# slcs-jsc/mptrac

Hardware: AMD Instinct MI355X
Metric: particle-steps/s (higher is better)
Workload: dtype f64

## Files before the change

### mptrac_amd/csrc/mphip_api.hip

```cpp
#include <hip/hip_runtime.h>
#include <dlfcn.h>
#include <unistd.h>

#include <algorithm>
#include <atomic>
#include <cmath>
#include <cstdio>
#include <cstring>
#include <string>
#include <mutex>
#include <thread>
#include <vector>

#include "mphip_buffers.hpp"
#include "mphip_kernels.hpp"
#include "mphip_metprep.hpp"
#include "mphip_regrid.hpp"
#include "mphip_detrend.hpp"
#include "mphip_ingest.hpp"
#include "mphip_pack.hpp"
#include "mphip_intpol.hpp"

using namespace mphip;

namespace {

constexpr unsigned kAdv = MPHIP_MOD_TIMESTEPS | MPHIP_MOD_POSITION | MPHIP_MOD_ADVECT | MPHIP_MOD_POSITION2;
constexpr unsigned kAdvTurb = kAdv | MPHIP_MOD_DIFF_TURB;
constexpr unsigned kAdvDiff = kAdvTurb | MPHIP_MOD_DIFF_MESO;
constexpr unsigned kAdvTurbConvSedi = kAdvTurb | MPHIP_MOD_CONVECTION | MPHIP_MOD_SEDI;
constexpr unsigned kAdvDiffConvSedi = kAdvDiff | MPHIP_MOD_CONVECTION | MPHIP_MOD_SEDI;
constexpr unsigned kDiffConvSediOnly = MPHIP_MOD_TIMESTEPS | MPHIP_MOD_DIFF_TURB | MPHIP_MOD_DIFF_MESO | MPHIP_MOD_CONVECTION
  | MPHIP_MOD_SEDI | MPHIP_MOD_POSITION2;
constexpr unsigned kTailOnly = MPHIP_MOD_TIMESTEPS;
constexpr unsigned kBound = MPHIP_MOD_BOUND_COND | MPHIP_MOD_BOUND_COND2;
constexpr unsigned kParticleBits = 0x3fffu | MPHIP_MOD_ISOSURF | kBound | MPHIP_MOD_ISOSURF_INIT;

const char *const kField3Name[MPHIP_N3D] = { "u", "v", "w", "t", "lwc", "rwc", "iwc", "swc", "pl", "ul", "vl", "zetal",
                                             "zeta_dotl", "h2o", "z", "pv", "o3", "cc", "wl" };
const char *const kField2Name[MPHIP_N2D] = { "ps", "pbl", "cape", "cin", "pel", "pct", "pcb", "cl", "ess", "nss", "shf", "ts",
                                             "zs", "us", "vs", "lsm", "sst", "pt", "tt", "zt", "h2ot", "plcl", "plfc", "o3c" };
// ... 69 lines not shown
    bool ml_monotonic = false;
    DevBuf<float> meso;
    bool meso_valid = false;
  };
  PackedGrids pk, pk_next;
  bool pk_next_valid = false;
  bool packed_dirty = true;

  long long np = 0, ip0 = 0, np_total = 0;
  int nq = 0;
  DevBuf<double> d_arr[4 + MPHIP_NQ_MAX];
  DevBuf<double> d_alt[4 + MPHIP_NQ_MAX];
  DevBuf<float> d_uvwp[3], d_uvwp_alt[3];
  DevBuf<double> d_dt, d_dt_alt;
  uint64_t rng_ctr = 0;
  DevBuf<double> d_iso, d_iso_alt;
  DevBuf<int> d_kz, d_kz_alt;
  DevBuf<double> d_iso_ts, d_iso_ps;
  int iso_n = 0;
  std::vector<std::pair<uintptr_t, uintptr_t>> pinned;
  std::mutex pinned_lock;

  DevBuf<int> d_ext, d_ext_alt;
  bool ext_identity = true;
  int steps_since_resort = 1 << 30;
  const int *fold_perm = nullptr;
  DevBuf<f32x4u> d_prec;

  DevBuf<uint32_t> d_keys[2];
  DevBuf<int> d_vals[2];
  DevBuf<uint32_t> d_counts;
  int sorted_buf = -1;
  const int *fused_perm = nullptr;
  bool fused_quantities = false;
  bool stored_is_sorted = false;
  long long sorted_n = 0;
  DevBuf<uint32_t> rep_sk, rep_mk[2], rep_fk, rep_tiles, rep_nm;
  DevBuf<int> rep_si, rep_mi[2], rep_fv;
  hipStream_t ahead_stream = nullptr;
  hipEvent_t ahead_mark = nullptr, ahead_done = nullptr;
  DevBuf<uint32_t> ahead_keys[2];
  DevBuf<int> ahead_vals[2];
  DevBuf<uint32_t> ahead_counts;
  DevBuf<double> ahead_dt;
  bool ahead_valid = false;
  double ahead_t = 0;
  int ahead_cur = 0;
  bool ahead_repaired = false;
  long long sorts_repaired = 0, sorts_scratch = 0;
  long long sorts_undone = 0;
  DevBuf<unsigned char> d_depo_busy;
  bool depo_busy_valid = false;
  const unsigned char *depo_busy_last = nullptr;
  unsigned depo_busy_last_mask = 0;

  DevBuf<int> d_cell;
  DevBuf<double> d_sums;
  DevBuf<int> d_cnt;
  DevBuf<unsigned long long> d_lists;
  DevBuf<double> d_rec;
  PinnedBuf<double> h_sums;
  DevBuf<double> d_grid_kernel;
  int grid_nk = 0;

  DevBuf<double> d_chemgrid;
  bool chemgrid_ok = false;
// ... 5 lines not shown
  RadioQnt radio = { { -1, -1, -1, -1, -1, -1 } };
  bool radio_on = false;
  bool rdepo_on = false;
  mphip_box_t rdepo_grid = {};
  DevBuf<double> d_rdepo_inv;
  size_t rdepo_ntot = 0;
  bool rdepo_have_t = false;
  double rdepo_t = 0;

  DevBuf<double> d_ana_kernel;
  DevBuf<uint32_t> d_marks;
  DevBuf<int> d_slot_of;
  DevBuf<uint32_t> d_ana_flags;

  mphip_allreduce_fn allreduce = nullptr;
  void *allreduce_user = nullptr;
  void *comm = nullptr;
  int comm_ranks = 1, comm_rank = 0;
  DevBuf<double> d_occ, d_band;
  PinnedBuf<double> h_occ;
  DevBuf<int> d_band_cnt;
  int mix_band_lo = -1, mix_band_hi = -1;

  PrepState prep;

  DevBuf<double> d_ip_in, d_ip_out;

  int locality_interval = 60;
  bool locality_zorder = false;
  int locality_tile = 0;
  int step_blocks = 8192;
  int step_blocks_multi = 32768;
  bool xcd_map = true;
  bool big_grid = false;
  bool force_generic = false;
  int multi_step = 64;
  bool fold_resort = true;
  int lds_tile = 0;
  bool turb_strat = true;
  bool compact_depo = true;
  bool pin_host_atm = false;
  bool perm_records = true;
  bool fuse_sort = true;
  bool fuse_quantities = true;
  int sort_bits = 0;
  bool sort_repair = true;
  bool sort_ahead = true;
  bool ahead_box = true;
  bool ahead_priority = false;
  bool emit_keys = true;
  int deterministic_sums = 1;
  int sum_path = 0;
  bool grid_records = true;
  int chain_blocks = 0;
  bool mix_exchange_levels = false;
  int derive_profile_phase = 0;
  int intpol_chunk = 1 << 22;

  bool prof = false;
  std::vector<hipEvent_t> ev;
  size_t ev_used = 0;
};

namespace {

int fail(mphip_ctx *ctx, const std::string &msg) {
// ... 654 lines not shown
      sel = kAdvDiffConvSedi | kGated | scheme | multi;
  } else if (!(rare_bits & ~kBound) && big_ok && (req & ~kOptionalModules) == kAdv) {
    sel = kAdvDiffConvSedi | kGated | kBigGrid | scheme | multi;
  }
#ifdef MPHIP_QUICK
  if (sel != kAdvDiffConvSedi && sel != (kAdvDiffConvSedi | kMultiStep) && sel != (kAdvDiffConvSedi | kMLWinds | kMultiStep)
      && sel != (kAdvDiffConvSedi | kGated | kPblClosure | kMultiStep))
    sel = kNoStepKernel;
#endif
  if (sel != kNoStepKernel)
    return sel;
  if (ml_fast)
    return nsteps > 1 ? kMaskGenericMLMulti : kMaskGenericML;
  if (nsteps > 1)
    return kNoStepKernel;
  return ml || (mask & kRareModules) || fg ? kMaskGeneric : kMaskGenericPL;
}

static bool reads_meso_table(unsigned sel, unsigned mask) {
  return sel != kNoStepKernel && sel < kMaskGenericMLMulti && (sel & MPHIP_MOD_DIFF_MESO)
    && !(sel & kBigGrid) && (mask & MPHIP_MOD_DIFF_MESO);
}

int ensure_meso_table(mphip_ctx *ctx) {
  mphip_ctx::PackedGrids &K = ctx->pk;
  if (K.meso_valid)
    return 0;
  HIPCHK(K.meso.reserve(meso_table_floats(ctx)));
  if (meso_table_launch(ctx, K, ctx->stream))
    return fail(ctx, "building the table of the mesoscale wind deviations failed");
  return 0;
}

int launch_step(mphip_ctx *ctx, unsigned mask, double t, const RngCtr &rng = {}, int nsteps = 1, double t_stride = 0,
                uint64_t ctr_stride = 0, const EmitKeys *emit = nullptr, bool *emitted = nullptr) {
  if (ctx->np == 0)
    return 0;
  if (ensure_packed(ctx) || check_fields(ctx, mask))
    return 1;
  if (ml_winds(ctx->ctl) && !ctx->d_kz.p) {
    const size_t n = (size_t) std::max<long long>(ctx->np, 1);
    HIPCHK(ctx->d_kz.resize(n));
    HIPCHK(ctx->d_kz_alt.resize(n));
    std::vector<int> mid(n, std::max(ctx->nml / 2, 0));
    HIPCHK(hipMemcpyAsync(ctx->d_kz.p, mid.data(), n * sizeof(int), hipMemcpyHostToDevice, ctx->stream));
    HIPCHK(hipStreamSynchronize(ctx->stream));
  }
  StepParams S;
  memset(&S.emit, 0, sizeof(S.emit));
  S.depo_busy = nullptr;
  if (emitted)
    *emitted = false;
  S.ctl = ctx->ctl;
  S.met = dev_met(ctx);
  S.atm = dev_atm(ctx);
  S.clim = ctx->d_clim.p;
  S.tracers = ctx->d_tracers.p;
  S.t = t;
  S.mask = mask;
  const BlockGeom geom = block_geom(ctx->np, nsteps > 1 ? ctx->step_blocks_multi : ctx->step_blocks);
  const int nb = geom.nblocks_logical;
  const long long per_block = geom.per_block;
  S.nblocks_logical = nb;
  S.per_block = per_block;
  S.xcd_map = ctx->xcd_map;
  S.ctr_turb = rng.turb;
  S.ctr_meso = rng.meso;
  S.ctr_conv = rng.conv;
  S.ctr_pbl = rng.pbl;
  S.radio = ctx->radio;
  S.nsteps = nsteps;
  S.t_stride = t_stride;
  S.ctr_stride = ctr_stride;
  size_t lds = axes_lds_bytes(ctx) + sizeof(DevClim) + (size_t) kLibmLogExpDoubles * sizeof(double);
  hipEvent_t e1 = nullptr;
  if (prof_pair(ctx, ctx->stream, &e1))
    return 1;
  unsigned sel = step_kernel_mask(ctx, mask, nsteps);
  if (reads_meso_table(sel, mask)) {
    if (ensure_meso_table(ctx))
      return 1;
    S.met.meso = ctx->pk.meso.p;
  }
  constexpr unsigned kDepo = MPHIP_MOD_WET_DEPO | MPHIP_MOD_DRY_DEPO;
  const size_t depo_lds = ((axes_lds_bytes(ctx) + 15) & ~(size_t) 15) + (size_t) per_block * sizeof(int);
  if (sel == kTailOnly && (mask & kDepo) && !(mask & ~kDepo) && ctx->compact_depo && !ctx->fused_perm
      && depo_lds <= 64 * 1024) {
    S.depo_busy = ctx->depo_busy_valid ? ctx->d_depo_busy.p : nullptr;
    ctx->depo_busy_valid = false;
    ctx->depo_busy_last = S.depo_busy;
    ctx->depo_busy_last_mask = mask;
    hipLaunchKernelGGL(depo_kernel, dim3(nb), dim3(256), depo_lds, ctx->stream, S);
    HIPCHK(hipGetLastError());
    ctx->fused_perm = nullptr;
    if (ctx->prof)
      HIPCHK(hipEventRecord(e1, ctx->stream));
    return 0;
  }
  ctx->depo_busy_valid = false;
  ctx->depo_busy_last = nullptr;
  if (emit && emit->keys && sel == kAdvDiffConvSedi && nsteps == 1) {
    sel |= kEmitKeys;
    S.emit = *emit;
    if (emitted)
      *emitted = true;
    ctx->depo_busy_valid = emit->depo_busy != nullptr;
  }
  if (ctx->lds_tile > 0 && nsteps > 1 && (sel == (kAdv | kMultiStep) || sel == (kAdv | kTwoStage | kMultiStep))
      && !(mask & (kTailModules | kBound)) && !ctx->fused_perm) {
    const size_t tile_lds = ((axes_lds_bytes(ctx) + 15) & ~(size_t) 15) + (size_t) ctx->lds_tile * 24;
    if (tile_lds <= 64 * 1024) {
      if (sel & kTwoStage)
        hipLaunchKernelGGL(traj_tile_kernel<2>, dim3(nb), dim3(256), tile_lds, ctx->stream, S, ctx->lds_tile);
      else
        hipLaunchKernelGGL(traj_tile_kernel<4>, dim3(nb), dim3(256), tile_lds, ctx->stream, S, ctx->lds_tile);
      HIPCHK(hipGetLastError());
      if (ctx->prof)
        HIPCHK(hipEventRecord(e1, ctx->stream));
      return 0;
    }
  }
  if (sel < kMaskGenericMLMulti && (sel & kPblClosure))
    lds += (size_t) (kLibmDoubles - kLibmLogExpDoubles) * sizeof(double);
  if (step_kernel_parks(sel))
    lds += kParkBytes;
  switch (sel) {
#define STEP_CASE(M)                                                                                  \
  case M:                                                                                             \
    hipLaunchKernelGGL(step_kernel<M>, dim3(nb), dim3(256), lds, ctx->stream, S);                     \
    break;
#ifdef MPHIP_QUICK
#define STEP_CASE_REST(M)
#else
#define STEP_CASE_REST(M) STEP_CASE(M)
#endif
    STEP_CASE_REST(kAdv)
    STEP_CASE_REST(kAdvTurb)
    STEP_CASE_REST(kAdvDiff)
    STEP_CASE_REST(kAdvTurbConvSedi)
    STEP_CASE(kAdvDiffConvSedi)
    STEP_CASE_REST(kAdv | kTwoStage)
    STEP_CASE_REST(kAdvTurb | kTwoStage)
    STEP_CASE_REST(kAdvDiff | kTwoStage)
    STEP_CASE_REST(kAdvTurbConvSedi | kTwoStage)
    STEP_CASE_REST(kAdvDiffConvSedi | kTwoStage)
    STEP_CASE_REST(kAdvDiffConvSedi | kGated)
    STEP_CASE_REST(kAdvDiffConvSedi | kGated | kTwoStage)
    STEP_CASE_REST(kTailOnly)
    STEP_CASE_REST(kDiffConvSediOnly)
    STEP_CASE_REST(kAdv | kMultiStep)
    STEP_CASE_REST(kAdvTurb | kMultiStep)
    STEP_CASE_REST(kAdvDiff | kMultiStep)
    STEP_CASE(kAdvDiffConvSedi | kMultiStep)
    STEP_CASE_REST(kAdvDiffConvSedi | kMLWinds)
    STEP_CASE(kAdvDiffConvSedi | kMLWinds | kMultiStep)
    STEP_CASE_REST(kAdvDiffConvSedi | kGated | kMLWinds)
    STEP_CASE_REST(kAdvDiffConvSedi | kGated | kMLWinds | kMultiStep)
    STEP_CASE_REST(kAdv | kTwoStage | kMultiStep)
    STEP_CASE_REST(kAdvTurb | kTwoStage | kMultiStep)
    STEP_CASE_REST(kAdvDiff | kTwoStage | kMultiStep)
    STEP_CASE_REST(kAdvDiffConvSedi | kTwoStage | kMultiStep)
    STEP_CASE_REST(kAdvDiffConvSedi | kGated | kMultiStep)
    STEP_CASE_REST(kAdvDiffConvSedi | kGated | kTwoStage | kMultiStep)
    STEP_CASE(kAdvDiffConvSedi | kEmitKeys)
    STEP_CASE_REST(kAdvDiffConvSedi | kGated | kPblClosure)
    STEP_CASE_REST(kAdvDiffConvSedi | kGated | kPblClosure | kTwoStage)
    STEP_CASE(kAdvDiffConvSedi | kGated | kPblClosure | kMultiStep)
    STEP_CASE_REST(kAdvDiffConvSedi | kGated | kPblClosure | kTwoStage | kMultiStep)
    STEP_CASE_REST(kAdvDiffConvSedi | kGated | kBigGrid)
    STEP_CASE_REST(kAdvDiffConvSedi | kGated | kBigGrid | kTwoStage)
    STEP_CASE_REST(kAdvDiffConvSedi | kGated | kBigGrid | kMultiStep)
    STEP_CASE_REST(kAdvDiffConvSedi | kGated | kBigGrid | kTwoStage | kMultiStep)
    STEP_CASE_REST(kAdvDiffConvSedi | kGated | kBigGrid | kMLWinds)
    STEP_CASE_REST(kAdvDiffConvSedi | kGated | kBigGrid | kMLWinds | kMultiStep)
    STEP_CASE(kMaskGeneric)
    STEP_CASE(kMaskGenericMLMulti)
    STEP_CASE(kMaskGenericML)
    STEP_CASE(kMaskGenericPL)
#undef STEP_CASE_REST
#undef STEP_CASE
  default:
    return fail(ctx, "internal: no multi-step instantiation for this module set");
  }
  HIPCHK(hipGetLastError());
  ctx->fused_perm = nullptr;
  if (ctx->prof)
    HIPCHK(hipEventRecord(e1, ctx->stream));
  return 0;
}


struct MeteoDeps {
  unsigned need3 = 0, need2 = 0;
};

MeteoDeps meteo_deps(const mphip_ctl_t &c) {
  MeteoDeps d;
  auto q = [&](int k) { return c.qnt_met[k] >= 0; };
  auto f3 = [&](int k, int f) { if (q(k)) d.need3 |= 1u << f; };
  auto f2 = [&](int k, int f) { if (q(k)) d.need2 |= 1u << f; };
  f2(MPHIP_MQ_PS, MPHIP_PS);     f2(MPHIP_MQ_TS, MPHIP_TS);     f2(MPHIP_MQ_ZS, MPHIP_ZS);
  f2(MPHIP_MQ_US, MPHIP_US);     f2(MPHIP_MQ_VS, MPHIP_VS);     f2(MPHIP_MQ_ESS, MPHIP_ESS);
  f2(MPHIP_MQ_NSS, MPHIP_NSS);   f2(MPHIP_MQ_SHF, MPHIP_SHF);   f2(MPHIP_MQ_LSM, MPHIP_LSM);
  f2(MPHIP_MQ_SST, MPHIP_SST);   f2(MPHIP_MQ_PBL, MPHIP_PBL);   f2(MPHIP_MQ_PT, MPHIP_PT);
  f2(MPHIP_MQ_TT, MPHIP_TT);     f2(MPHIP_MQ_ZT, MPHIP_ZT);     f2(MPHIP_MQ_H2OT, MPHIP_H2OT);
  f2(MPHIP_MQ_PCT, MPHIP_PCT);   f2(MPHIP_MQ_PCB, MPHIP_PCB);   f2(MPHIP_MQ_CL, MPHIP_CL);
  f2(MPHIP_MQ_PLCL, MPHIP_PLCL); f2(MPHIP_MQ_PLFC, MPHIP_PLFC); f2(MPHIP_MQ_PEL, MPHIP_PEL);
  f2(MPHIP_MQ_CAPE, MPHIP_CAPE); f2(MPHIP_MQ_CIN, MPHIP_CIN);   f2(MPHIP_MQ_O3C, MPHIP_O3C);
  f3(MPHIP_MQ_ZG, MPHIP_Z);      f3(MPHIP_MQ_T, MPHIP_T);       f3(MPHIP_MQ_U, MPHIP_U);
  f3(MPHIP_MQ_V, MPHIP_V);       f3(MPHIP_MQ_W, MPHIP_W);       f3(MPHIP_MQ_H2O, MPHIP_H2O);
  f3(MPHIP_MQ_O3, MPHIP_O3);     f3(MPHIP_MQ_LWC, MPHIP_LWC);   f3(MPHIP_MQ_RWC, MPHIP_RWC);
  f3(MPHIP_MQ_IWC, MPHIP_IWC);   f3(MPHIP_MQ_SWC, MPHIP_SWC);   f3(MPHIP_MQ_CC, MPHIP_CC);
  f3(MPHIP_MQ_PV, MPHIP_PV);
  f3(MPHIP_MQ_RHO, MPHIP_T);     f3(MPHIP_MQ_VH, MPHIP_U);      f3(MPHIP_MQ_VH, MPHIP_V);
  f3(MPHIP_MQ_VZ, MPHIP_W);      f3(MPHIP_MQ_PSAT, MPHIP_T);    f3(MPHIP_MQ_PSICE, MPHIP_T);
  f3(MPHIP_MQ_PW, MPHIP_H2O);    f3(MPHIP_MQ_SH, MPHIP_H2O);    f3(MPHIP_MQ_RH, MPHIP_T);
// ... 1126 lines not shown
    if (reserve(ctx, ctx->d_rec, (size_t) ctx->np * (size_t) nv) || reserve(ctx, ctx->d_sums, (size_t) nv * ntot))
      return 1;
    R.cell = ctx->d_cell.p;
    R.val = ctx->d_rec.p;
    StepParams S;
    memset(&S.emit, 0, sizeof(S.emit));
    S.ctl = c;
    S.met = dev_met(ctx);
    S.atm = dev_atm(ctx);
    S.clim = ctx->d_clim.p;
    S.tracers = ctx->d_tracers.p;
    S.t = t;
    S.mask = depo;
    int blocks = ctx->step_blocks;
    BlockGeom geom = block_geom(ctx->np, blocks);
    const size_t axes = (axes_lds_bytes(ctx) + 15) & ~(size_t) 15;
    const size_t lds_max = 64 * 1024 - 8;
    while (axes + (size_t) geom.per_block * sizeof(int) > lds_max && geom.per_block > 256) {
      blocks *= 2;
      geom = block_geom(ctx->np, blocks);
    }
    const size_t lds = axes + (size_t) geom.per_block * sizeof(int);
    if (lds > lds_max)
      return fail(ctx, "module_radio_depo: the axes of the meteo grid do not fit the LDS");
    S.nblocks_logical = geom.nblocks_logical;
    S.per_block = geom.per_block;
    S.xcd_map = ctx->xcd_map;
    S.depo_busy = busy;
    S.ctr_turb = S.ctr_meso = S.ctr_conv = S.ctr_pbl = 0;
    S.radio = ctx->radio;
    S.nsteps = 1;
    S.t_stride = 0;
    S.ctr_stride = 0;
    hipEvent_t e1 = nullptr;
    if (prof_pair(ctx, ctx->stream, &e1))
      return 1;
    hipLaunchKernelGGL(radio_depo_kernel, dim3(geom.nblocks_logical), dim3(256), lds, ctx->stream, S, R);
    HIPCHK(hipGetLastError());
    if (ctx->prof)
      HIPCHK(hipEventRecord(e1, ctx->stream));
    const RecordVals vals = { ctx->d_rec.p, nv };
    if (ordered_cell_sums(ctx, vals, nv, 1, ntot, ctx->d_sums.p, (int *) nullptr, (double *) nullptr, true))
      return 1;
    step = ctx->d_sums.p;
  }
  ctx->rdepo_t = t;
  ctx->rdepo_have_t = true;
  if (D.ndep > 0) {
    hipLaunchKernelGGL(radio_depo_add_kernel, dim3(grid_for((long long) (2 * (size_t) D.ndep * ntot))), dim3(256), 0, ctx->stream,
                       ctx->d_rdepo_inv.p, step, ntot, D);
    HIPCHK(hipGetLastError());
  }
  return 0;
}

int launch_chem(mphip_ctx *ctx, double t) {
  const mphip_ctl_t &c = ctx->ctl;
  return (chem_on(c)
          && (do_chem_grid(ctx, t) || (c.oh_chem_reaction != 0 && launch_oh(ctx))
              || (c.h2o2_chem_reaction != 0 && launch_h2o2(ctx))))
    || (c.tracer_chem != 0 && launch_tracer_chem(ctx));
}


struct StepDue {
  bool sort, mixing, conv, meteo;
// ... 3175 lines not shown

int flush_if_switched_off(mphip_ctx *ctx, double value) {
  return value == 0 ? flush_meteo(ctx) : 0;
}

int drop_sort_ahead(mphip_ctx *ctx, double) {
  return ahead_drop(ctx);
}

int resort_next_step(mphip_ctx *ctx, double) {
  ctx->steps_since_resort = 1 << 30;
  return 0;
}

const char *const kStepBlocksRefusal = "step_blocks must be in 8 ... 1048576";

const Option kOptions[] = {
  number("locality_sort_interval", &mphip_ctx::locality_interval, kRange, 0, HUGE_VAL, "locality_sort_interval must be >= 0"),
  number("step_blocks", &mphip_ctx::step_blocks, kRange, 8, 1048576, kStepBlocksRefusal),
  number("step_blocks_multi", &mphip_ctx::step_blocks_multi, kRange, 8, 1048576, kStepBlocksRefusal),
  flag("fuse_sort", &mphip_ctx::fuse_sort),
  flag("lazy_meteo", &mphip_ctx::lazy_meteo, flush_if_switched_off),
  flag("pin_host_atm", &mphip_ctx::pin_host_atm),
  number("multi_step", &mphip_ctx::multi_step, kRange, 0, 4096, "multi_step must be in 0 ... 4096"),
  flag("fold_resort", &mphip_ctx::fold_resort),
  flag("turb_strat", &mphip_ctx::turb_strat),
  flag("fuse_sort_quantities", &mphip_ctx::fuse_quantities),
  flag("perm_records", &mphip_ctx::perm_records),
  flag("big_grid", &mphip_ctx::big_grid),
  number("derive_profile_phase", &mphip_ctx::derive_profile_phase, kWhole, 0, 6,
         "derive_profile_phase must be 0 (kernels), 1 (uploads), 2 (downloads), 3 (the weight table of "
         "mphip_detrend_met) or 4, 5, 6 (the extremes, their reduction, the quantisation of mphip_pack_met)"),
  flag("xcd_map", &mphip_ctx::xcd_map),
  flag("generic_kernel", &mphip_ctx::force_generic),
  number("sort_bits", &mphip_ctx::sort_bits, kZeroOrRange, 8, kRadixMaxBits, "sort_bits must be 0 (automatic), 8, 9 or 10"),
  flag("mix_exchange_levels", &mphip_ctx::mix_exchange_levels),
  number("lds_tile", &mphip_ctx::lds_tile, kZeroOrRange, 64, 2400, "lds_tile must be 0 or 64 ... 2400 cells"),
  flag("ahead_priority", &mphip_ctx::ahead_priority),
  flag("emit_keys", &mphip_ctx::emit_keys),
  flag("sort_repair", &mphip_ctx::sort_repair),
  flag("compact_depo", &mphip_ctx::compact_depo),
  flag("ahead_box", &mphip_ctx::ahead_box),
  flag("sort_ahead", &mphip_ctx::sort_ahead, drop_sort_ahead),
  number("sum_path", &mphip_ctx::sum_path, kWhole, 0, 2, "sum_path must be 0, 1 or 2"),
  number("deterministic_sums", &mphip_ctx::deterministic_sums, kWhole, 0, 1, "deterministic_sums must be 0 or 1"),
  flag("grid_records", &mphip_ctx::grid_records),
  number("chain_blocks", &mphip_ctx::chain_blocks, kRange, -HUGE_VAL, HUGE_VAL, nullptr),
  flag("locality_zorder", &mphip_ctx::locality_zorder, resort_next_step),
  number("locality_tile", &mphip_ctx::locality_tile, kRange, 0, 64, "locality_tile must be in 0 ... 64", resort_next_step),
  number("intpol_chunk", &mphip_ctx::intpol_chunk, kRange, 64, 1 << 24, "intpol_chunk must be in 64 ... 16777216"),
};

}

int mphip_set_option(mphip_ctx *ctx, const char *name, double value) {
  if (!ctx || !name)
    return 1;
  for (const Option &o : kOptions) {
    if (strcmp(name, o.name) != 0)
      continue;
    const bool inside = value >= o.lo && value <= o.hi;
    if ((o.kind == kRange && (value < o.lo || value > o.hi)) || (o.kind == kZeroOrRange && !(value == 0 || inside))
        || (o.kind == kWhole && !(inside && value == std::floor(value))))
      return fail(ctx, o.refusal);
    if (o.before && o.before(ctx, value))
      return 1;
// ... 87 lines not shown
  HIPCHK(hipGetLastError());
  HIPCHK(hipMemcpyAsync(out, dout.p, (size_t) n * sizeof(double), hipMemcpyDeviceToHost, ctx->stream));
  HIPCHK(hipStreamSynchronize(ctx->stream));
  return 0;
}

int mphip_test_piece(mphip_ctx *ctx, int piece, int reps, double *checksum) {
  if (!ctx || !ctx->have_ctl || ctx->np == 0)
    return fail(ctx, "mphip_test_piece needs control parameters and particles");
  HIPCHK(hipSetDevice(ctx->device));
  if (ensure_packed(ctx))
    return 1;
  if (!ctx->have_clim)
    return fail(ctx, "climatological tropopause data were not uploaded");
  StepParams S;
  memset(&S.emit, 0, sizeof(S.emit));
  S.depo_busy = nullptr;
  S.ctl = ctx->ctl;
  S.met = dev_met(ctx);
  S.atm = dev_atm(ctx);
  S.clim = ctx->d_clim.p;
  S.tracers = ctx->d_tracers.p;
  S.t = 0;
  S.mask = 0;
  const BlockGeom geom = block_geom(ctx->np, ctx->step_blocks);
  const int nb = geom.nblocks_logical;
  S.nblocks_logical = nb;
  S.per_block = geom.per_block;
  S.xcd_map = ctx->xcd_map;
  S.ctr_turb = 1000;
  S.ctr_meso = 5000;
  S.ctr_conv = 9000;
  S.ctr_pbl = 0;
  if (piece == 22) {
    if (!lean32_ok(ctx))
      return fail(ctx, "mphip_test_piece: piece 22 needs a grid the lean kernels with 32-bit offsets run on");
    if (ensure_meso_table(ctx))
      return 1;
    S.met.meso = ctx->pk.meso.p;
  }
  DevBuf<double> out;
  HIPCHK(out.resize((size_t) ctx->np));
  double *const d = out.p;
  const size_t lds = axes_lds_bytes(ctx) + sizeof(DevClim) + (size_t) kLibmLogExpDoubles * sizeof(double);
  switch (piece) {
#define PIECE_CASE(K)                                                                                  \
  case K:                                                                                              \
    hipLaunchKernelGGL(piece_kernel<K>, dim3(nb), dim3(256), lds, ctx->stream, S, reps, d);            \
    break;
#ifdef MPHIP_QUICK
    PIECE_CASE(0)
#else
    PIECE_CASE(0) PIECE_CASE(1) PIECE_CASE(2) PIECE_CASE(3) PIECE_CASE(4) PIECE_CASE(5) PIECE_CASE(6) PIECE_CASE(7)
    PIECE_CASE(8) PIECE_CASE(9) PIECE_CASE(10) PIECE_CASE(11) PIECE_CASE(12) PIECE_CASE(13) PIECE_CASE(14)
    PIECE_CASE(15) PIECE_CASE(16) PIECE_CASE(17) PIECE_CASE(18) PIECE_CASE(19) PIECE_CASE(20) PIECE_CASE(21)
    PIECE_CASE(22) PIECE_CASE(23) PIECE_CASE(24) PIECE_CASE(25) PIECE_CASE(26)
#endif
#undef PIECE_CASE
  default:
    return fail(ctx, "unknown piece");
  }
  HIPCHK(hipGetLastError());
  HIPCHK(hipStreamSynchronize(ctx->stream));
  if (checksum) {
    std::vector<double> h((size_t) std::min<long long>(ctx->np, 1024));
    HIPCHK(hipMemcpy(h.data(), d, h.size() * sizeof(double), hipMemcpyDeviceToHost));
// ... 50 lines not shown
```

### mptrac_amd/csrc/mphip_kernels.hpp

```cpp
#pragma once

#include <type_traits>
#include "mphip_device.hpp"

namespace mphip {



struct BoxGrid {
  double lon0, lon1, lat0, lat1, z0, z1;
  int nx, ny, nz;
};

constexpr int kMixMax = 8 + MPHIP_NRADIO;
struct MixSet {
  double *q[kMixMax];
  int n;
};

__device__ __forceinline__ int box_cell(const BoxGrid &G, double t0, double t1, double time, double lon, double lat,
                                        double p, const double *__restrict__ ens, long long i, int ngrid) {
  const double dz = (G.z1 - G.z0) / G.nz;
  const double dlon = (G.lon1 - G.lon0) / G.nx;
  const double dlat = (G.lat1 - G.lat0) / G.ny;
// ... 53 lines not shown
}

struct EmitKeys {
  uint32_t *keys;
  double *dt_next;
  int *cell;
  BoxGrid grid;
  double box_t0, box_t1;
  const double *ens;
  int ngrid;
  double direction, t_start, t_stop, t_next;
  unsigned char *depo_busy;
  unsigned depo_mask;
};

struct StepParams {
  EmitKeys emit;
  mphip_ctl_t ctl;
  DevMet met;
  DevAtm atm;
  const DevClim *clim;
  const DevTracerSeries *tracers;
  double t;
  unsigned mask;
  int nblocks_logical;
  long long per_block;
  int xcd_map;
  const unsigned char *depo_busy;
  uint64_t ctr_turb, ctr_meso, ctr_conv, ctr_pbl;
  RadioQnt radio;
  int nsteps;
  double t_stride;
  uint64_t ctr_stride;
};

template <class Params>
__device__ __forceinline__ void block_range(const Params &G, long long np, long long &first, long long &last) {
  const int nb = G.nblocks_logical;
  const int lb = G.xcd_map ? (int) (blockIdx.x % 8) * (nb / 8) + (int) (blockIdx.x / 8) : (int) blockIdx.x;
  first = (long long) lb * G.per_block;
  last = first + G.per_block;
  if (last > np)
    last = np;
}

constexpr unsigned kMaskGeneric = 0xffffffffu;
constexpr unsigned kMaskGenericPL = 0xfffffffeu;
constexpr unsigned kMaskGenericML = 0xfffffffdu;
constexpr unsigned kMaskGenericMLMulti = 0xfffffffbu;
template <unsigned CT>
constexpr bool kGenericML = (CT == kMaskGenericML || CT == kMaskGenericMLMulti);
template <unsigned CT>
constexpr bool kRuntimeMask = (CT == kMaskGeneric || CT == kMaskGenericPL || kGenericML<CT>);
constexpr unsigned kMLWinds = 1u << 27;
template <unsigned CT>
constexpr bool kLeanML = !kRuntimeMask<CT> && (CT & kMLWinds) != 0;
constexpr unsigned kBigGrid = 1u << 28;
template <unsigned CT>
constexpr bool kBig = !kRuntimeMask<CT> && (CT & kBigGrid) != 0;
template <unsigned CT>
constexpr bool kModelLevels = kGenericML<CT> || kLeanML<CT>;
constexpr unsigned kRareModules = MPHIP_MOD_ADVECT_INIT | MPHIP_MOD_ISOSURF_INIT | MPHIP_MOD_ISOSURF | MPHIP_MOD_DIFF_PBL
  | MPHIP_MOD_BOUND_COND | MPHIP_MOD_BOUND_COND2;
constexpr unsigned kStoreDt = 1u << 30;
constexpr unsigned kTwoStage = 1u << 24;
constexpr unsigned kGated = 1u << 25;
constexpr unsigned kMultiStep = 1u << 26;
constexpr unsigned kPblClosure = 1u << 29;
constexpr unsigned kEmitKeys = 1u << 22;
constexpr unsigned kTemplateFlags = kTwoStage | kGated | kMultiStep | kMLWinds | kBigGrid | kPblClosure | kEmitKeys;
constexpr unsigned kOptionalModules = MPHIP_MOD_DIFF_TURB | MPHIP_MOD_DIFF_MESO | MPHIP_MOD_CONVECTION | MPHIP_MOD_SEDI;
constexpr unsigned kRadioDecay = 1u << 31;
constexpr unsigned kTailModules = MPHIP_MOD_LOSS_ZERO | MPHIP_MOD_DECAY | kRadioDecay | MPHIP_MOD_WET_DEPO | MPHIP_MOD_DRY_DEPO;
constexpr unsigned kMovers = MPHIP_MOD_POSITION | MPHIP_MOD_ADVECT | MPHIP_MOD_DIFF_TURB | MPHIP_MOD_DIFF_MESO | MPHIP_MOD_DIFF_PBL
  | MPHIP_MOD_CONVECTION | MPHIP_MOD_SEDI | MPHIP_MOD_ISOSURF | MPHIP_MOD_POSITION2;

// ... 271 lines not shown
  return ct < kMaskGenericMLMulti && (ct & kMultiStep) && !(ct & (kMLWinds | kPblClosure))
    && (ct & (MPHIP_MOD_DIFF_TURB | MPHIP_MOD_DIFF_MESO | MPHIP_MOD_CONVECTION | MPHIP_MOD_SEDI));
}
struct PermRest {
  float up, vp, wp;
  int ext;
};
__device__ __forceinline__ PermRest perm_rest(const DevAtm &a, long long i, long long src, bool store_uvwp) {
  PermRest r;
  a.dt[i] = a.s_dt[src];
  r.ext = a.s_ext ? a.s_ext[src] : (int) src;
  a.ext_out[i] = r.ext;
  r.up = a.s_up[src];
  r.vp = a.s_vp[src];
  r.wp = a.s_wp[src];
  if (store_uvwp) {
    a.up[i] = r.up;
    a.vp[i] = r.vp;
    a.wp[i] = r.wp;
  }
  return r;
}
__device__ __attribute__((noinline)) PermRest perm_rest_call(const DevAtm *a, long long i, long long src, bool store_uvwp) {
  return perm_rest(*a, i, src, store_uvwp);
}

constexpr bool step_kernel_stores_once(unsigned ct) {
  return ct != 0 && ct < kMaskGenericMLMulti && (ct & kMultiStep) && !(ct & kMLWinds);
}
constexpr int kParkDoubles = 256 * 2 + 128;
constexpr size_t kParkBytes = kParkDoubles * sizeof(double);
enum { kParkRp = 0, kParkRhop = 256, kParkExt = 512 };
template <class T>
__device__ __forceinline__ T *park_slot(double *area, int slot, long long i) {
  unsigned lane = (unsigned) i & 255u;
  asm volatile("" : "+v"(lane));
  return (T *) (area + slot) + lane;
}

template <unsigned CT>
__global__ __launch_bounds__(256, kLeanML<CT> ? MPHIP_ML_WAVES_PER_SIMD : !kRuntimeMask<CT> && (CT & kPblClosure) ? MPHIP_PBL_WAVES_PER_SIMD : !kRuntimeMask<CT> ? ((CT & kMultiStep) ? MPHIP_MULTI_WAVES_PER_SIMD
                                                        : (CT & MPHIP_MOD_ADVECT) || CT == MPHIP_MOD_TIMESTEPS ? MPHIP_LEAN_WAVES_PER_SIMD : MPHIP_SPLITB_WAVES_PER_SIMD)
                                   : (CT == kMaskGenericPL ? MPHIP_STEP_WAVES_PER_SIMD : MPHIP_GENERIC_WAVES_PER_SIMD)) void step_kernel(
  const StepParams S) {
  extern __shared__ double s_lds[];
  constexpr bool park = step_kernel_parks(CT);
  double *const s_axes = s_lds + (park ? kParkDoubles : 0);
  const unsigned mask = kRuntimeMask<CT> ? S.mask : (CT & ~kTemplateFlags);
  using MLCol = std::conditional_t<kLeanML<CT> && !kBig<CT>, uint32_t, size_t>;
  const DevMet &M = S.met;
  const DevAtm &a = S.atm;
  const mphip_ctl_t &ctl = S.ctl;

  const Axes A = load_axes(M, s_axes);
  const DevClim *clim = S.clim;
  if ((mask | (kRuntimeMask<CT> ? 0u : (S.mask & kTailModules))) & (MPHIP_MOD_DIFF_TURB | MPHIP_MOD_DECAY)) {
    double *dst = s_axes + ((axes_doubles(M) * 8 + (size_t) M.lut_size * 2 + 15) & ~(size_t) 15) / 8;
    const double *src = (const double *) S.clim;
    for (int i = threadIdx.x; i < (int) (sizeof(DevClim) / sizeof(double)); i += blockDim.x)
      dst[i] = src[i];
    clim = (const DevClim *) dst;
  }
  const double *ltab = libm_tables();
  if (!kRuntimeMask<CT> && (mask & (MPHIP_MOD_DIFF_TURB | MPHIP_MOD_DIFF_MESO | MPHIP_MOD_SEDI))) {
    double *dst = s_axes + ((axes_doubles(M) * 8 + (size_t) M.lut_size * 2 + 15) & ~(size_t) 15) / 8
      + sizeof(DevClim) / sizeof(double);
    const double *src = libm_tables();
    for (int i = threadIdx.x; i < ((CT & kPblClosure) ? kLibmDoubles : kLibmLogExpDoubles); i += blockDim.x)
      dst[i] = src[i];
    ltab = dst;
  }
  __syncthreads();

  long long first, last;
  block_range(S, a.np, first, last);

  for (long long i = first + threadIdx.x; i < last; i += (park ? 256 : blockDim.x)) {
    auto kp = (const __attribute__((address_space(4))) StepParams *) __builtin_amdgcn_kernarg_segment_ptr();
    asm volatile("" : "+s"(kp));
    const StepParams &S = *(const StepParams *) kp;
    const DevMet &M = S.met;
    const DevAtm &a = S.atm;
    const mphip_ctl_t &ctl = S.ctl;
    constexpr bool multi = (!kRuntimeMask<CT> && (CT & kMultiStep) != 0) || CT == kMaskGenericMLMulti;
    const int nsteps = multi ? S.nsteps : 1;
    double t_now = S.t;
    uint64_t c_turb = S.ctr_turb, c_meso = S.ctr_meso, c_conv = S.ctr_conv, c_pbl = S.ctr_pbl;
    constexpr bool store_once = multi && !kRuntimeMask<CT> && !kModelLevels<CT>;
    static_assert(store_once == step_kernel_stores_once(CT), "step_kernel_stores_once");
    Particle P;
    WindCache wc;
    float up = 0.f, vp = 0.f, wp = 0.f;
    for (int step = 0; step < nsteps; step++, t_now += S.t_stride, c_turb += S.ctr_stride, c_meso += S.ctr_stride,
             c_conv += S.ctr_stride, c_pbl += S.ctr_stride) {
    const bool fused_sort = a.perm != nullptr;
    if (!multi || step == 0) {
    constexpr bool perm_call = store_once && (CT & kPblClosure) != 0;
    const bool perm_all = store_once && !perm_call && fused_sort && a.perm_all;
    if (fused_sort) {
      const long long src = a.perm[i];
      if constexpr (perm_call)
        if (a.perm_all)
          (void) perm_rest_call(&a, i, src, true);
      P.time = a.s_time[src];
      P.lon = a.s_lon[src];
      P.lat = a.s_lat[src];
      P.p = a.s_p[src];
      for (int k = 0; k < a.nq_perm; k++)
        a.q[k][i] = a.s_q[k][src];
      if constexpr (store_once && !perm_call) {
        if (a.perm_all) {
          const PermRest r = perm_rest(a, i, src, !(mask & MPHIP_MOD_DIFF_MESO));
          if constexpr (park)
            *park_slot<int>(s_lds, kParkExt, i) = r.ext;
          up = r.up;
          vp = r.vp;
          wp = r.wp;
        }
      }
    } else {
      P.time = a.time[i];
      P.lon = a.lon[i];
      P.lat = a.lat[i];
      P.p = a.p[i];
    }
    if (multi && (mask & MPHIP_MOD_DIFF_MESO) && !perm_all) {
      up = a.up[i];
      vp = a.vp[i];
      wp = a.wp[i];
    }
    if constexpr (park) {
      if (a.ext && !perm_all)
        *park_slot<int>(s_lds, kParkExt, i) = a.ext[i];
      if (((CT & kGated) ? mask & S.mask : mask) & MPHIP_MOD_SEDI) {
        *park_slot<double>(s_lds, kParkRp, i) = a.q[ctl.qnt_rp][i];
        *park_slot<double>(s_lds, kParkRhop, i) = a.q[ctl.qnt_rhop][i];
      }
    }
    }
    if (CT == kMaskGeneric && (mask & (MPHIP_MOD_ADVECT_INIT | MPHIP_MOD_ISOSURF_INIT))) {
      P.dt = 0;
      if (mask & MPHIP_MOD_ISOSURF_INIT)
        a.iso[i] = isosurf_value(ctl, M, A, P);
      if (mask & MPHIP_MOD_ADVECT_INIT)
        a.p[i] = pressure_from_zeta(M, A, P.time, a.q[ctl.qnt_zeta][i], P.lon, P.lat);
      continue;
    }
    if (kModelLevels<CT> && (mask & MPHIP_MOD_ADVECT_INIT)) {
      a.p[i] = pressure_from_zeta_fast(M, A, P.time, a.q[ctl.qnt_zeta][i], P.lon, P.lat);
      continue;
    }
    if (S.mask & MPHIP_MOD_TIMESTEPS) {
      P.dt = timestep_of(ctl, M, A, P.time, P.lon, P.lat, t_now);
      if (S.mask & kStoreDt)
        a.dt[i] = P.dt;
    } else
      P.dt = a.dt[i];
    if (P.dt == 0) {
      if (fused_sort && !store_once) {
        a.time[i] = P.time;
        a.lon[i] = P.lon;
        a.lat[i] = P.lat;
        a.p[i] = P.p;
      }
      if (CT == kMaskGeneric && (mask & MPHIP_MOD_ISOSURF))
        a.p[i] = isosurf_pressure(ctl, M, A, a, P, ctl.isosurf <= 3 ? a.iso[i] : 0.0);
      if constexpr (!kRuntimeMask<CT> && (CT & kEmitKeys) != 0)
        if (S.emit.keys)
          emit_sort_keys(S.emit, ctl, M, A, i, P);
      if constexpr (!kRuntimeMask<CT> && (CT & kPblClosure) != 0)
        if (S.mask & MPHIP_MOD_ISOSURF) {
          P.p = isosurf_call(&ctl, &M, A, &a, P.time, P.p, P.lon, P.lat, ctl.isosurf <= 3 ? a.iso[i] : 0.0);
          if (!store_once)
            a.p[i] = P.p;
        }
      continue;
    }
    const uint64_t g_held = park ? 0 : (uint64_t) (a.ip0 + (a.ext ? (long long) a.ext[i] : i));
    auto g_now = [&]() -> uint64_t {
      if constexpr (park)
        return (uint64_t) (a.ip0 + (a.ext ? (long long) *park_slot<int>(s_lds, kParkExt, i) : i));
      else
        return g_held;
    };

    constexpr bool lean = !kRuntimeMask<CT>;
    if (!kModelLevels<CT>)
      wind_cache_reset(wc, CT != kMaskGeneric && (lean || !MPHIP_EXACT_DIV));
    if (mask & MPHIP_MOD_POSITION) {
      if (lean)
        position_fast(M, A, P);
      else
        position(M, A, P);
    }
    if (mask & MPHIP_MOD_ADVECT) {
      if (CT == kMaskGeneric && ctl.advect_vert_coord == 2) {
        advect_mlp(ctl, M, A, P);
      } else if (kModelLevels<CT> && ctl.advect_vert_coord == 2) {
        int kz = a.kz[i];
        advect_mlp_fast<MLCol>(ctl, M, A, P, kz);
        a.kz[i] = kz;
      } else if (CT == kMaskGeneric && (ctl.advect_vert_coord == 1 || ctl.advect_vert_coord == 3)) {
        const int qnt = ctl.advect_vert_coord == 1 ? ctl.qnt_zeta : ctl.qnt_eta;
        double zeta;
        advect_ml(ctl, M, A, P, zeta);
        a.q[qnt][i] = zeta;
      } else if (kModelLevels<CT>) {
        const int qnt = ctl.advect_vert_coord == 1 ? ctl.qnt_zeta : ctl.qnt_eta;
        double zeta;
        int kz = a.kz[i];
        advect_ml_fast<MLCol>(ctl, M, A, P, zeta, kz);
        a.kz[i] = kz;
        a.q[qnt][i] = zeta;
      } else if (lean && (CT & kTwoStage))
// ... 29 lines not shown
        vp = st.vp;
        wp = st.wp;
        wind_cache_reset(wc, true);
      } else
        diff_pbl<false>(M, A, P, up, vp, wp, c_pbl, g_now(), ltab);
      if (!(store_once && held)) {
        a.up[i] = up;
        a.vp[i] = vp;
        a.wp[i] = wp;
      }
    }
    if (opt & MPHIP_MOD_DIFF_MESO) {
      if (!multi) {
        up = a.up[i];
        vp = a.vp[i];
        wp = a.wp[i];
      }
      if (kGenericML<CT>)
        wind_cache_reset(wc, true);
      if (lean)
        diff_meso_fast<!(CT & MPHIP_MOD_ADVECT) || kLeanML<CT>, kBig<CT>>(ctl, M, A, P, up, vp, wp, c_meso, g_now(), wc, ltab);
      else
        diff_meso(ctl, M, A, P, up, vp, wp, c_meso, g_now(), wc, ltab);
      if (!store_once) {
        a.up[i] = up;
        a.vp[i] = vp;
        a.wp[i] = wp;
      }
    }
    if (lean) {
      if (opt & (MPHIP_MOD_CONVECTION | MPHIP_MOD_SEDI)) {
        const bool sedi_on = (opt & MPHIP_MOD_SEDI) != 0;
        conv_sedi_fast<kBig<CT>>(ctl, M, A, P, opt, c_conv, g_now(),
                       !sedi_on ? 0.0 : park ? *park_slot<double>(s_lds, kParkRp, i) : a.q[ctl.qnt_rp][i],
                       !sedi_on ? 0.0 : park ? *park_slot<double>(s_lds, kParkRhop, i) : a.q[ctl.qnt_rhop][i], ltab);
      }
    } else {
      if (opt & MPHIP_MOD_CONVECTION)
        convection(ctl, M, A, P, c_conv, g_now());
      if (opt & MPHIP_MOD_SEDI)
        sedimentation(M, A, P, a.q[ctl.qnt_rp][i], a.q[ctl.qnt_rhop][i]);
    }
    if (CT == kMaskGeneric && (mask & MPHIP_MOD_ISOSURF))
      P.p = isosurf_pressure(ctl, M, A, a, P, ctl.isosurf <= 3 ? a.iso[i] : 0.0);
    if constexpr (lean && (CT & kPblClosure) != 0)
      if (S.mask & MPHIP_MOD_ISOSURF)
        P.p = isosurf_call(&ctl, &M, A, &a, P.time, P.p, P.lon, P.lat, ctl.isosurf <= 3 ? a.iso[i] : 0.0);
    if (mask & MPHIP_MOD_POSITION2) {
      if (lean)
        position_fast(M, A, P);
      else
        position(M, A, P);
    }

    if (!store_once) {
      if ((mask & MPHIP_MOD_ADVECT) || fused_sort)
        a.time[i] = P.time;
      if ((mask & kMovers) || fused_sort) {
        a.lon[i] = P.lon;
        a.lat[i] = P.lat;
        a.p[i] = P.p;
      }
    }
    if constexpr (lean && (CT & kEmitKeys) != 0)
      if (S.emit.keys)
        emit_sort_keys(S.emit, ctl, M, A, i, P);

    constexpr bool bound_rt = lean && ((CT & kGated) || (CT & ~kTemplateFlags) == MPHIP_MOD_TIMESTEPS);
// ... 11 lines not shown
    }
    if (tmask & kRadioDecay)
      radio_decay(S.radio, a, i, P.dt, ltab);
    if (lean) {
      const bool wet = (tmask & MPHIP_MOD_WET_DEPO) && !above_every_cloud_top(M, P);
      const bool dry = (tmask & MPHIP_MOD_DRY_DEPO) && !above_every_surface_layer(ctl, M, P);
      if (wet || dry) {
        Stencil sd = stencil_zero();
        horiz_fast(M, A, P.lon, P.lat, sd);
        depo_pair_fast<kBig<CT>>(ctl, M, A, a, i, P, sd, wet, dry);
      }
    } else {
      if (mask & MPHIP_MOD_WET_DEPO)
        wet_depo(ctl, M, A, a, i, P);
      if (mask & MPHIP_MOD_DRY_DEPO)
        dry_depo(ctl, M, A, a, i, P);
    }
    if (bmask & MPHIP_MOD_BOUND_COND2)
      bound_cond(ctl, M, A, a, i, P, S.tracers);
    }
    if constexpr (store_once) {
      static_assert((CT & MPHIP_MOD_ADVECT) != 0, "a lean multi-step instantiation without the advection");
      a.time[i] = P.time;
      a.lon[i] = P.lon;
      a.lat[i] = P.lat;
      a.p[i] = P.p;
      if (mask & MPHIP_MOD_DIFF_MESO) {
        a.up[i] = up;
        a.vp[i] = vp;
        a.wp[i] = wp;
      }
    }
  }
}

#ifndef MPHIP_TILE_WAVES_PER_SIMD
#define MPHIP_TILE_WAVES_PER_SIMD 3
#endif
template <int STAGES>
__global__ __launch_bounds__(256, MPHIP_TILE_WAVES_PER_SIMD) void traj_tile_kernel(const StepParams S, int tile_cells) {
  extern __shared__ double s_axes[];
  __shared__ int s_lo[3], s_hi[3];
  const DevMet &M = S.met;
  const DevAtm &a = S.atm;
  const mphip_ctl_t &ctl = S.ctl;
  const Axes A = load_axes(M, s_axes);
  float *s_tile = (float *) (s_axes + ((axes_doubles(M) * 8 + (size_t) M.lut_size * 2 + 15) & ~(size_t) 15) / 8);
  long long first, last;
  block_range(S, a.np, first, last);
  for (long long base = first; base < last; base += 256) {
    const long long i = base + threadIdx.x;
    const bool live = i < last;
    if (threadIdx.x < 3) {
      s_lo[threadIdx.x] = 1 << 30;
      s_hi[threadIdx.x] = -1;
    }
    __syncthreads();
    Particle P;
    P.time = P.lon = P.lat = P.p = P.dt = 0;
    int lo[3] = { 1 << 30, 1 << 30, 1 << 30 }, hi[3] = { -1, -1, -1 };
    if (live) {
      P.time = a.time[i];
      P.lon = a.lon[i];
      P.lat = a.lat[i];
      P.p = a.p[i];
      Stencil s0;
// ... 2482 lines not shown
```

Before: 14.78 billion.

## Distribute step-kernel work via per-XCD atomic chunk queues sized to resident blocks

Replaces the static per-block particle ranges in the step kernel with a persistent-style grid, sized from the occupancy query, whose waves claim 64-particle chunks from atomic counters. There is one counter per XCD, and the last wave to finish resets the counters. The aim is to balance load across waves when per-particle cost varies and to cut launch tail imbalance. In exchange it adds an atomic per chunk, changes the particle-to-wave mapping, which may hurt memory locality, and needs the LDS park slots to be re-indexed by wave. By default (step_queue=1) it only engages when there are enough chunks per wave.

```diff
diff --git a/mptrac_amd/csrc/mphip_api.hip b/mptrac_amd/csrc/mphip_api.hip
--- a/mptrac_amd/csrc/mphip_api.hip
+++ b/mptrac_amd/csrc/mphip_api.hip
@@ -7,6 +7,7 @@
 #include <cmath>
 #include <cstdio>
 #include <cstring>
+#include <map>
 #include <string>
 #include <mutex>
 #include <thread>
@@ -142,6 +143,8 @@
   DevBuf<uint32_t> d_counts;
   int sorted_buf = -1;
   const int *fused_perm = nullptr;
+  DevBuf<int> d_step_queue;
+  std::map<std::pair<const void *, size_t>, int> step_resident;
   bool fused_quantities = false;
   bool stored_is_sorted = false;
   long long sorted_n = 0;
@@ -213,6 +216,7 @@
   int step_blocks = 8192;
   int step_blocks_multi = 32768;
   bool xcd_map = true;
+  int step_queue = 1;
   bool big_grid = false;
   bool force_generic = false;
   int multi_step = 64;
@@ -933,6 +937,35 @@
   return 0;
 }
 
+constexpr int kQueueChunksPerWave = 16;
+int step_queue_grid(mphip_ctx *ctx, void (*kernel)(const StepParams), size_t lds, int blocks, StepParams &S, int *grid) {
+  if (ctx->step_queue == 0)
+    return 0;
+  const auto key = std::make_pair((const void *) kernel, lds);
+  auto it = ctx->step_resident.find(key);
+  if (it == ctx->step_resident.end()) {
+    int per_cu = 0, cus = 0;
+    HIPCHK(hipOccupancyMaxActiveBlocksPerMultiprocessor(&per_cu, kernel, 256, lds));
+    HIPCHK(hipDeviceGetAttribute(&cus, hipDeviceAttributeMultiprocessorCount, ctx->device));
+    it = ctx->step_resident.emplace(key, std::max(per_cu, 1) * std::max(cus, 1)).first;
+  }
+  const long long nchunks = (ctx->np + 63) / 64;
+  long long g = std::max<long long>(8, std::min(it->second, blocks) & ~7);
+  if (nchunks > 0x7fffffffll || (ctx->step_queue == 1 && nchunks < (long long) kQueueChunksPerWave * kStepWaves * g))
+    return 0;
+  g = std::min(g, ((nchunks + kStepWaves - 1) / kStepWaves + 7) & ~7ll);
+  if (!ctx->d_step_queue.p) {
+    HIPCHK(ctx->d_step_queue.resize(kQueueInts));
+    HIPCHK(hipMemsetAsync(ctx->d_step_queue.p, 0, kQueueInts * sizeof(int), ctx->stream));
+  }
+  S.queue = ctx->d_step_queue.p;
+  S.queue_n = ctx->xcd_map ? 8 : 1;
+  S.queue_chunks = (int) ((nchunks + S.queue_n - 1) / S.queue_n);
+  S.queue_waves = (int) g * kStepWaves;
+  *grid = (int) g;
+  return 0;
+}
+
 int launch_step(mphip_ctx *ctx, unsigned mask, double t, const RngCtr &rng = {}, int nsteps = 1, double t_stride = 0,
                 uint64_t ctr_stride = 0, const EmitKeys *emit = nullptr, bool *emitted = nullptr) {
   if (ctx->np == 0)
@@ -973,6 +1006,8 @@
   S.nsteps = nsteps;
   S.t_stride = t_stride;
   S.ctr_stride = ctr_stride;
+  S.queue = nullptr;
+  S.queue_n = S.queue_chunks = S.queue_waves = 0;
   size_t lds = axes_lds_bytes(ctx) + sizeof(DevClim) + (size_t) kLibmLogExpDoubles * sizeof(double);
   hipEvent_t e1 = nullptr;
   if (prof_pair(ctx, ctx->stream, &e1))
@@ -1025,10 +1060,11 @@
     lds += (size_t) (kLibmDoubles - kLibmLogExpDoubles) * sizeof(double);
   if (step_kernel_parks(sel))
     lds += kParkBytes;
+  void (*kernel)(const StepParams) = nullptr;
   switch (sel) {
 #define STEP_CASE(M)                                                                                  \
   case M:                                                                                             \
-    hipLaunchKernelGGL(step_kernel<M>, dim3(nb), dim3(256), lds, ctx->stream, S);                     \
+    kernel = step_kernel<M>;                                                                          \
     break;
 #ifdef MPHIP_QUICK
 #define STEP_CASE_REST(M)
@@ -1083,6 +1119,10 @@
   default:
     return fail(ctx, "internal: no multi-step instantiation for this module set");
   }
+  int grid = nb;
+  if (step_queue_grid(ctx, kernel, lds, nsteps > 1 ? ctx->step_blocks_multi : ctx->step_blocks, S, &grid))
+    return 1;
+  hipLaunchKernelGGL(kernel, dim3(grid), dim3(256), lds, ctx->stream, S);
   HIPCHK(hipGetLastError());
   ctx->fused_perm = nullptr;
   if (ctx->prof)
@@ -2275,6 +2315,8 @@
     S.nsteps = 1;
     S.t_stride = 0;
     S.ctr_stride = 0;
+    S.queue = nullptr;
+    S.queue_n = S.queue_chunks = S.queue_waves = 0;
     hipEvent_t e1 = nullptr;
     if (prof_pair(ctx, ctx->stream, &e1))
       return 1;
@@ -5516,6 +5558,7 @@
          "derive_profile_phase must be 0 (kernels), 1 (uploads), 2 (downloads), 3 (the weight table of "
          "mphip_detrend_met) or 4, 5, 6 (the extremes, their reduction, the quantisation of mphip_pack_met)"),
   flag("xcd_map", &mphip_ctx::xcd_map),
+  number("step_queue", &mphip_ctx::step_queue, kWhole, 0, 2, "step_queue must be 0, 1 or 2"),
   flag("generic_kernel", &mphip_ctx::force_generic),
   number("sort_bits", &mphip_ctx::sort_bits, kZeroOrRange, 8, kRadixMaxBits, "sort_bits must be 0 (automatic), 8, 9 or 10"),
   flag("mix_exchange_levels", &mphip_ctx::mix_exchange_levels),
@@ -5669,6 +5712,8 @@
   S.ctr_meso = 5000;
   S.ctr_conv = 9000;
   S.ctr_pbl = 0;
+  S.queue = nullptr;
+  S.queue_n = S.queue_chunks = S.queue_waves = 0;
   if (piece == 22) {
     if (!lean32_ok(ctx))
       return fail(ctx, "mphip_test_piece: piece 22 needs a grid the lean kernels with 32-bit offsets run on");
diff --git a/mptrac_amd/csrc/mphip_kernels.hpp b/mptrac_amd/csrc/mphip_kernels.hpp
--- a/mptrac_amd/csrc/mphip_kernels.hpp
+++ b/mptrac_amd/csrc/mphip_kernels.hpp
@@ -109,6 +109,8 @@
   int nsteps;
   double t_stride;
   uint64_t ctr_stride;
+  int *queue;
+  int queue_n, queue_chunks, queue_waves;
 };
 
 template <class Params>
@@ -119,6 +121,69 @@
   last = first + G.per_block;
   if (last > np)
     last = np;
+}
+
+constexpr int kQueueStride = 32;
+constexpr int kQueueDone = 8;
+constexpr int kQueueInts = (kQueueDone + 1) * kQueueStride;
+constexpr int kStepWaves = 4;
+
+__device__ __forceinline__ const StepParams &step_kernarg() {
+  auto kp = (const __attribute__((address_space(4))) StepParams *) __builtin_amdgcn_kernarg_segment_ptr();
+  asm volatile("" : "+s"(kp));
+  return *(const StepParams *) kp;
+}
+__device__ __forceinline__ int wave_lane() {
+  int lane;
+  asm volatile("v_mbcnt_lo_u32_b32 %0, -1, 0\n\tv_mbcnt_hi_u32_b32 %0, -1, %0" : "=v"(lane));
+  return lane;
+}
+typedef unsigned ChunkWalk;
+__device__ __forceinline__ int chunk_claim(ChunkWalk &walk) {
+  const StepParams &S = step_kernarg();
+  const int nq = S.queue_n, per = S.queue_chunks;
+  const int nchunks = (int) ((S.atm.np + 63) >> 6);
+  for (; (int) (walk & 15u) < nq; walk++) {
+    const int q = (int) (((walk >> 4) + walk) & (unsigned) (nq - 1));
+    const int begin = q * per;
+    const int n = nchunks - begin < per ? nchunks - begin : per;
+    if (n <= 0)
+      continue;
+    int c = 0;
+    if (wave_lane() == 0)
+      c = atomicAdd(S.queue + q * kQueueStride, 1);
+    c = __builtin_amdgcn_readfirstlane(c);
+    if (c < n)
+      return begin + c;
+  }
+  return -1;
+}
+__device__ __forceinline__ int chunk_first(ChunkWalk &walk) {
+  const StepParams &S = step_kernarg();
+  const unsigned wave = (unsigned) __builtin_amdgcn_readfirstlane((int) threadIdx.x) >> 6;
+  if (S.queue_n) {
+    walk = wave << 30 | (blockIdx.x & 7u) << 4;
+    return chunk_claim(walk);
+  }
+  long long first, last;
+  block_range(S, S.atm.np, first, last);
+  const int end = (int) ((last + 63) >> 6);
+  walk = wave << 30 | (unsigned) end;
+  const int c = (int) (first >> 6) + (int) wave;
+  return c < end ? c : -1;
+}
+__device__ __forceinline__ int chunk_next(long long i, ChunkWalk &walk) {
+  if (step_kernarg().queue_n)
+    return chunk_claim(walk);
+  const int c = __builtin_amdgcn_readfirstlane((int) (i >> 6)) + kStepWaves;
+  return c < (int) (walk & 0x3fffffffu) ? c : -1;
+}
+__device__ __forceinline__ void chunk_walk_end() {
+  const StepParams &S = step_kernarg();
+  if (S.queue_n && wave_lane() == 0
+      && atomicAdd(S.queue + kQueueDone * kQueueStride, 1) == S.queue_waves - 1)
+    for (int q = 0; q <= kQueueDone; q++)
+      __hip_atomic_store(S.queue + q * kQueueStride, 0, __ATOMIC_RELAXED, __HIP_MEMORY_SCOPE_AGENT);
 }
 
 constexpr unsigned kMaskGeneric = 0xffffffffu;
@@ -456,8 +521,9 @@
 constexpr size_t kParkBytes = kParkDoubles * sizeof(double);
 enum { kParkRp = 0, kParkRhop = 256, kParkExt = 512 };
 template <class T>
-__device__ __forceinline__ T *park_slot(double *area, int slot, long long i) {
-  unsigned lane = (unsigned) i & 255u;
+__device__ __forceinline__ T *park_slot(double *area, int slot, ChunkWalk walk, long long i) {
+  asm volatile("" : "+s"(walk));
+  unsigned lane = ((unsigned) i & 63u) | ((walk >> 24) & 0xc0u);
   asm volatile("" : "+v"(lane));
   return (T *) (area + slot) + lane;
 }
@@ -496,10 +562,12 @@
   }
   __syncthreads();
 
-  long long first, last;
-  block_range(S, a.np, first, last);
-
-  for (long long i = first + threadIdx.x; i < last; i += (park ? 256 : blockDim.x)) {
+  ChunkWalk walk;
+  long long i;
+  for (int chunk = chunk_first(walk); chunk >= 0; chunk = chunk_next(i, walk)) {
+    i = 64ll * chunk + wave_lane();
+    if (i >= step_kernarg().atm.np)
+      continue;
     auto kp = (const __attribute__((address_space(4))) StepParams *) __builtin_amdgcn_kernarg_segment_ptr();
     asm volatile("" : "+s"(kp));
     const StepParams &S = *(const StepParams *) kp;
@@ -536,7 +604,7 @@
         if (a.perm_all) {
           const PermRest r = perm_rest(a, i, src, !(mask & MPHIP_MOD_DIFF_MESO));
           if constexpr (park)
-            *park_slot<int>(s_lds, kParkExt, i) = r.ext;
+            *park_slot<int>(s_lds, kParkExt, walk, i) = r.ext;
           up = r.up;
           vp = r.vp;
           wp = r.wp;
@@ -555,10 +623,10 @@
     }
     if constexpr (park) {
       if (a.ext && !perm_all)
-        *park_slot<int>(s_lds, kParkExt, i) = a.ext[i];
+        *park_slot<int>(s_lds, kParkExt, walk, i) = a.ext[i];
       if (((CT & kGated) ? mask & S.mask : mask) & MPHIP_MOD_SEDI) {
-        *park_slot<double>(s_lds, kParkRp, i) = a.q[ctl.qnt_rp][i];
-        *park_slot<double>(s_lds, kParkRhop, i) = a.q[ctl.qnt_rhop][i];
+        *park_slot<double>(s_lds, kParkRp, walk, i) = a.q[ctl.qnt_rp][i];
+        *park_slot<double>(s_lds, kParkRhop, walk, i) = a.q[ctl.qnt_rhop][i];
       }
     }
     }
@@ -603,7 +671,7 @@
     const uint64_t g_held = park ? 0 : (uint64_t) (a.ip0 + (a.ext ? (long long) a.ext[i] : i));
     auto g_now = [&]() -> uint64_t {
       if constexpr (park)
-        return (uint64_t) (a.ip0 + (a.ext ? (long long) *park_slot<int>(s_lds, kParkExt, i) : i));
+        return (uint64_t) (a.ip0 + (a.ext ? (long long) *park_slot<int>(s_lds, kParkExt, walk, i) : i));
       else
         return g_held;
     };
@@ -699,8 +767,8 @@
       if (opt & (MPHIP_MOD_CONVECTION | MPHIP_MOD_SEDI)) {
         const bool sedi_on = (opt & MPHIP_MOD_SEDI) != 0;
         conv_sedi_fast<kBig<CT>>(ctl, M, A, P, opt, c_conv, g_now(),
-                       !sedi_on ? 0.0 : park ? *park_slot<double>(s_lds, kParkRp, i) : a.q[ctl.qnt_rp][i],
-                       !sedi_on ? 0.0 : park ? *park_slot<double>(s_lds, kParkRhop, i) : a.q[ctl.qnt_rhop][i], ltab);
+                       !sedi_on ? 0.0 : park ? *park_slot<double>(s_lds, kParkRp, walk, i) : a.q[ctl.qnt_rp][i],
+                       !sedi_on ? 0.0 : park ? *park_slot<double>(s_lds, kParkRhop, walk, i) : a.q[ctl.qnt_rhop][i], ltab);
       }
     } else {
       if (opt & MPHIP_MOD_CONVECTION)
@@ -778,6 +846,7 @@
       }
     }
   }
+  chunk_walk_end();
 }
 
 #ifndef MPHIP_TILE_WAVES_PER_SIMD
```

Result: faster. 15.74 billion (median of 6 runs) (+6.5%).
